# MIT-SPARK/BUFFER-X

Hardware: NVIDIA H100
Metric: registration pairs/sec (20k-pt clouds, 1500 kpts, 50k RANSAC) (higher is better)
Workload: dtype f32

## Files before the change

### buffer-x_b200/csrc/bx_conv_sd.cu

```cuda
#include <cuda_fp16.h>

#include "bx_common.cuh"
#include "bx_wgmma.cuh"

namespace {

constexpr int SD_BM = 128;
constexpr int SD_AROWS = 176;
constexpr int SD_SROWS = 176;
constexpr int SD_KBYTES = SD_AROWS * 16;
constexpr int SD_CHUNK = 4 * SD_KBYTES;
constexpr int SD_NL = 3;
constexpr int SD_NC = 8;
constexpr int SD_WGT_WARP = SD_NC + 3;
constexpr int SD_MAXNA = 12, SD_MAXNBS = 24;
constexpr int SD_TRING = 32;
constexpr int SD_SMEM = 227 * 1024 - 2048;

struct ConvSdParams {
    const float *in;
    const __half *w;
    const float *bias;
    float *out;
    int *flag;
    int n, Cout, nchunks, is3d, S_in, G_in, relu, n_tiles, NA;
    const int *d_n;
    const float *fa, *fb;
    int cyl, rs, W, OD, OW, S_out, rs_out;
    const __half *in_sd;
    __half *out_sd;
    long long rows_in, rows_out;
    int nbs;
    int resident;
    int *tile_ctr;
};

template <int NT, int IN_SD> struct SdCfg {
    static constexpr int NB = (NT == 128 && !IN_SD) ? 64 : NT;
    static constexpr int NH = NT / NB;
    static constexpr int SB = NT < 64 ? NT : 64;
    static constexpr int THREADS = (SD_NC + 4) * 32;
    static constexpr int PROD_REGS = IN_SD ? 56 : 136, MMA_REGS = IN_SD ? 224 : 184;
    static constexpr int B_STAGE = 3 * 64 * NT;
    static constexpr int STAGE_BYTES = SD_BM * SB * 4;
};
static_assert(128 * SdCfg<64, 1>::PROD_REGS + 256 * SdCfg<64, 1>::MMA_REGS == 384 * 168, "register split of the presplit kernels");
static_assert(128 * SdCfg<64, 0>::PROD_REGS + 256 * SdCfg<64, 0>::MMA_REGS == 384 * 168, "register split of the fp32-input kernels");

template <int R> __device__ __forceinline__ void setmaxnreg_inc() { asm volatile("setmaxnreg.inc.sync.aligned.u32 %0;" ::"n"(R)); }
template <int R> __device__ __forceinline__ void setmaxnreg_dec() { asm volatile("setmaxnreg.dec.sync.aligned.u32 %0;" ::"n"(R)); }

template <int CW, int OUT_SD, class Get8>
__device__ __forceinline__ void sd_store_rows(const ConvSdParams &p, int t, int row, int co0, int n_samples, Get8 get8) {
    const uint32_t R = (uint32_t)t * SD_BM + (uint32_t)row;
    const uint32_t s = R / (uint32_t)p.rs, q = R - s * (uint32_t)p.rs;
    const uint32_t y = q / (uint32_t)p.W, x = q - y * (uint32_t)p.W;
    const bool live = (int)s < n_samples;
    const bool valid = live && (int)y < p.OD && (int)x < p.OW;
    if constexpr (!OUT_SD) {
        if (!valid) return;
        const int S_out = p.S_out;
        float4 *eo = reinterpret_cast<float4 *>(p.out) + ((size_t)s * (p.Cout >> 2) + (co0 >> 2)) * S_out + (y * p.OW + x);
#pragma unroll
        for (int c = 0; c < CW; c += 8) {
            float r[8];
            get8(c, r);
#pragma unroll
            for (int e = 0; e < 8; ++e) r[e] = p.relu ? fmaxf(r[e], 0.0f) : r[e];
            if (co0 + c < p.Cout) eo[(size_t)(c >> 2) * S_out] = make_float4(r[0], r[1], r[2], r[3]);
            if (co0 + c + 4 < p.Cout) eo[(size_t)((c >> 2) + 1) * S_out] = make_float4(r[4], r[5], r[6], r[7]);
        }
    } else {
        const bool wz = p.cyl && live && ((y == 7 && x <= 20) || (y == 6 && x == 21));
        const bool z0 = p.cyl && R < 22;
        if (!valid && !wz && !z0) return;
        const size_t rows = (size_t)p.rows_out;
        const size_t pmain = p.cyl ? (size_t)R + 23 : (size_t)s * p.rs_out + y * p.OW + x;
        const long long pdup = !p.cyl ? -1 : (x == 19 ? (long long)R + 3 : (x == 0 ? (long long)R + 43 : -1));
        uint4 *img = reinterpret_cast<uint4 *>(p.out_sd) + (size_t)((co0 >> 4) * 4 + ((co0 >> 3) & 1)) * rows;
        const uint4 z = make_uint4(0u, 0u, 0u, 0u);
        float omax = 0.0f;
#pragma unroll
        for (int c = 0; c < CW; c += 8) {
            if (co0 + c < p.Cout) {
                if (valid) {
                    float r[8];
                    get8(c, r);
                    uint32_t hi[4], lo[4];
#pragma unroll
                    for (int e = 0; e < 4; ++e) {
                        float a = r[2 * e], b = r[2 * e + 1];
                        if (p.relu) { a = fmaxf(a, 0.0f); b = fmaxf(b, 0.0f); }
                        const __half2 hh = __floats2half2_rn(a, b);
                        const float2 hf = __half22float2(hh);
                        const __half2 ll = __floats2half2_rn((a - hf.x) * 2048.0f, (b - hf.y) * 2048.0f);
                        hi[e] = *reinterpret_cast<const uint32_t *>(&hh);
                        lo[e] = *reinterpret_cast<const uint32_t *>(&ll);
                        omax = fmaxf(omax, fmaxf(fabsf(a), fabsf(b)));
                    }
                    const uint4 vh = make_uint4(hi[0], hi[1], hi[2], hi[3]), vl = make_uint4(lo[0], lo[1], lo[2], lo[3]);
                    img[pmain] = vh; img[2 * rows + pmain] = vl;
                    if (pdup >= 0) { img[pdup] = vh; img[2 * rows + pdup] = vl; }
                } else if (wz) { img[pmain] = z; img[2 * rows + pmain] = z; }
                if (z0) { img[R] = z; img[2 * rows + R] = z; }
            }
            img += (((co0 + c) >> 3) & 1) ? 3 * rows : rows;
        }
        if (!(omax < 65000.0f) && p.flag) atomicOr(p.flag, 1);
    }
}

template <int NT, int IN_SD, int OUT_SD>
__global__ void __launch_bounds__(SdCfg<NT, IN_SD>::THREADS, 1) conv_sd_kernel(const ConvSdParams p) {
    using C = SdCfg<NT, IN_SD>;
    constexpr int NB = C::NB, NH = C::NH, SB = C::SB, WGT_WARP = SD_WGT_WARP;
    constexpr int BAR_AFULL = 0, BAR_AEMPTY = SD_MAXNA, BAR_BFULL = 2 * SD_MAXNA, BAR_BEMPTY = BAR_BFULL + SD_MAXNBS;
    constexpr int BAR_TILE = BAR_BEMPTY + SD_MAXNBS, NBARS = BAR_TILE + SD_TRING;
    extern __shared__ __align__(128) unsigned char smem[];
    __shared__ __align__(8) unsigned long long bars[NBARS];
    __shared__ int tile_ring[SD_TRING];
    __shared__ __align__(16) float bias_s[128];

    const int tid = threadIdx.x, lane = tid & 31;
    const int warp = __shfl_sync(0xffffffffu, tid >> 5, 0);
    const int NA = p.NA, NBS = p.nbs, nchunks = p.nchunks;
    const bool resident = p.resident != 0;
    const int n_samples = p.d_n ? min(*p.d_n, p.n) : p.n;
    const int n_tiles = (int)(((long long)n_samples * p.rs + SD_BM - 1) / SD_BM);
    float *const stage = reinterpret_cast<float *>(smem + (size_t)NA * SD_CHUNK + (size_t)NBS * C::B_STAGE);

    if (tid == 0) {
        for (int s = 0; s < SD_MAXNA; ++s) {
            mbar_init(smem_u32(&bars[BAR_AFULL + s]), IN_SD ? 1 : SD_NL);
            mbar_init(smem_u32(&bars[BAR_AEMPTY + s]), SD_NC);
        }
        for (int s = 0; s < SD_MAXNBS; ++s) {
            mbar_init(smem_u32(&bars[BAR_BFULL + s]), 1);
            mbar_init(smem_u32(&bars[BAR_BEMPTY + s]), SD_NC);
        }
        for (int s = 0; s < SD_TRING; ++s) mbar_init(smem_u32(&bars[BAR_TILE + s]), 1);
        asm volatile("fence.mbarrier_init.release.cluster;" ::: "memory");
    }
    if (threadIdx.x < 128) bias_s[threadIdx.x] = (int)threadIdx.x < p.Cout ? __ldg(p.bias + threadIdx.x) : 0.0f;
    __syncthreads();
    uint32_t a_base = smem_u32(smem);
    uint32_t b_base = a_base + (uint32_t)NA * SD_CHUNK;
    uint32_t bar_base = smem_u32(&bars[0]);
    asm volatile("" : "+r"(a_base), "+r"(b_base), "+r"(bar_base));

    const bool dyn = IN_SD && p.tile_ctr != nullptr;
    auto tile_of = [&](uint32_t k) -> int {
        if (!dyn) { const long long t = (long long)blockIdx.x + (long long)k * gridDim.x; return t < n_tiles ? (int)t : -1; }
        mbar_wait(bar_base + 8u * (BAR_TILE + (k & (SD_TRING - 1))), (k / SD_TRING) & 1u);
        return tile_ring[k & (SD_TRING - 1)];
    };

    if (warp < SD_NC) {
        setmaxnreg_inc<C::MMA_REGS>();
        const int wg = warp >> 2, tl = tid & 127;
        const int r0 = wg * 64 + (warp & 3) * 16 + (lane >> 2);
        const int cq = 2 * (lane & 3);
        constexpr uint32_t DESC_HI = 128u >> 4;
        constexpr uint32_t A_LBO = ((uint32_t)SD_KBYTES >> 4) << 16;
        constexpr uint32_t B_LBO = ((uint32_t)(2 * NT * 16) >> 4) << 16;
        constexpr uint32_t A_SPLIT = (2u * SD_KBYTES) >> 4, B_TAP16 = (64u * NT) >> 4, B_LO16 = (uint32_t)(NT * 16) >> 4;
        const uint32_t a0 = ((a_base + (uint32_t)wg * 64u * 16u) >> 4) | A_LBO;
        const uint32_t b0 = (b_base >> 4) | B_LBO;
        const uint32_t Wrow = (uint32_t)p.W;
        float run[NT / 2], acc[NB];
        uint32_t slot = 0, a_par = 0, q = 0, k = 0;
        for (int t = tile_of(0); t >= 0; t = tile_of(++k)) {
#pragma unroll
            for (int i = 0; i < NT / 2; ++i) run[i] = bias_s[(i / (NB / 2)) * NB + 8 * ((i % (NB / 2)) >> 2) + cq + (i & 1)];
            for (int c = 0; c < nchunks; ++c) {
                mbar_wait(bar_base + 8u * (BAR_AFULL + slot), a_par);
                const uint32_t ac = a0 + slot * ((uint32_t)SD_CHUNK >> 4);
                const uint32_t q0 = resident ? (uint32_t)c * 3u : q;
#pragma unroll
                for (int h = 0; h < NH; ++h) {
                    wgmma_fence();
#pragma unroll
                    for (int g = 0; g < 3; ++g) {
                        const uint32_t sq = q0 + (uint32_t)g, sb = sq % (uint32_t)NBS;
                        if (h == 0) mbar_wait(bar_base + 8u * (BAR_BFULL + sb), resident ? 0u : (sq / (uint32_t)NBS) & 1u);
                        const uint32_t bg = b0 + sb * ((uint32_t)C::B_STAGE >> 4);
#pragma unroll
                        for (int tt = 0; tt < 3; ++tt) {
                            const uint32_t ah = ac + (uint32_t)g * Wrow + (uint32_t)tt, al = ah + A_SPLIT;
                            const uint32_t bh = bg + (uint32_t)tt * B_TAP16 + (uint32_t)(h * NB), bl = bh + B_LO16;
                            const uint32_t acc_on = (g == 0 && tt == 0) ? 0u : 1u;
                            wgmma_f16<NB>(acc, gmma_desc(ah, DESC_HI), gmma_desc(bh, DESC_HI), acc_on);
                            if constexpr (NT < 128) {
                                wgmma_f16<NB>(acc + NB / 2, gmma_desc(ah, DESC_HI), gmma_desc(bl, DESC_HI), acc_on);
                                wgmma_f16<NB>(acc + NB / 2, gmma_desc(al, DESC_HI), gmma_desc(bh, DESC_HI), 1u);
                            } else {
                                wgmma_f16<NB>(acc + NB / 2, gmma_desc(al, DESC_HI), gmma_desc(bh, DESC_HI), acc_on);
                                wgmma_f16<NB>(acc + NB / 2, gmma_desc(ah, DESC_HI), gmma_desc(bl, DESC_HI), 1u);
                            }
                        }
                    }
                    wgmma_commit();
                    wgmma_wait<0>();
                    wgmma_fence_regs<NB>(acc);
#pragma unroll
                    for (int i = 0; i < NB / 2; ++i) run[h * (NB / 2) + i] += fmaf(acc[NB / 2 + i], 0.00048828125f, acc[i]);
                }
                __syncwarp();
                if (lane == 0) {
                    mbar_arrive(bar_base + 8u * (BAR_AEMPTY + slot));
                    if (!resident)
                        for (int g = 0; g < 3; ++g) mbar_arrive(bar_base + 8u * (BAR_BEMPTY + (q0 + (uint32_t)g) % (uint32_t)NBS));
                }
                if (++slot == (uint32_t)NA) { slot = 0; a_par ^= 1u; }
                if (!resident) q += 3;
            }
#pragma unroll
            for (int h = 0; h < NT / SB; ++h) {
                asm volatile("bar.sync %0, 128;" ::"r"(1 + wg) : "memory");
#pragma unroll
                for (int i = 0; i < SB / 2; i += 2) {
                    const int col = 8 * (i >> 2) + cq, row = r0 + ((i & 2) ? 8 : 0);
                    *reinterpret_cast<float2 *>(stage + ((size_t)(col >> 2) * SD_BM + row) * 4 + (col & 3)) =
                        make_float2(run[h * (SB / 2) + i], run[h * (SB / 2) + i + 1]);
                }
                asm volatile("bar.sync %0, 128;" ::"r"(1 + wg) : "memory");
                const int row = wg * 64 + (tl & 63), cs = (tl >> 6) * (SB / 2);
                const float4 *st4 = reinterpret_cast<const float4 *>(stage);
                sd_store_rows<SB / 2, OUT_SD>(p, t, row, h * SB + cs, n_samples, [&](int cc, float (&r)[8]) {
                    const float4 u0 = st4[((cs + cc) >> 2) * SD_BM + row], u1 = st4[(((cs + cc) >> 2) + 1) * SD_BM + row];
                    r[0] = u0.x; r[1] = u0.y; r[2] = u0.z; r[3] = u0.w; r[4] = u1.x; r[5] = u1.y; r[6] = u1.z; r[7] = u1.w;
                });
            }
        }
    } else {
        setmaxnreg_dec<C::PROD_REGS>();
        if (warp < WGT_WARP) {
            if (IN_SD) {
                if (warp == SD_NC && lane == 0) {
                    uint32_t slot = 0, par = 0, round = 0;
                    for (uint32_t k = 0;; ++k) {
                        int t;
                        if (dyn) {
                            t = atomicAdd(p.tile_ctr, 1);
                            if (t >= n_tiles) t = -1;
                            tile_ring[k & (SD_TRING - 1)] = t;
                            mbar_arrive(bar_base + 8u * (BAR_TILE + (k & (SD_TRING - 1))));
                        } else {
                            t = tile_of(k);
                        }
                        if (t < 0) break;
                        for (int c = 0; c < nchunks; ++c) {
                            if (round) mbar_wait(bar_base + 8u * (BAR_AEMPTY + slot), par ^ 1u);
                            mbar_arrive_expect_tx(bar_base + 8u * (BAR_AFULL + slot), 4u * (uint32_t)SD_KBYTES);
                            const unsigned char *src = reinterpret_cast<const unsigned char *>(p.in_sd) + ((size_t)(c * 4) * p.rows_in + (size_t)t * SD_BM) * 16;
#pragma unroll
                            for (int im = 0; im < 4; ++im)
                                bulk_g2s(a_base + slot * (uint32_t)SD_CHUNK + (uint32_t)im * SD_KBYTES, src + (size_t)im * p.rows_in * 16, (uint32_t)SD_KBYTES,
                                         bar_base + 8u * (BAR_AFULL + slot));
                            if (++slot == (uint32_t)NA) { slot = 0; par ^= 1u; round = 1; }
                        }
                    }
                }
                __syncwarp();
            } else {
                constexpr int ITEMS = (2 * SD_AROWS + SD_NL * 32 - 1) / (SD_NL * 32);
                const int ltid = tid - SD_NC * 32;
                const float4 *in4 = reinterpret_cast<const float4 *>(p.in);
                float amax = 0.0f;
                float4 cur[ITEMS][2], nxt[ITEMS][2];
                auto issue = [&](int t, int c, float4 (&v)[ITEMS][2]) {
                    const long long p0 = (long long)t * SD_BM;
#pragma unroll
                    for (int m = 0; m < ITEMS; ++m) {
                        const int idx = ltid + m * SD_NL * 32;
                        v[m][0] = make_float4(0.f, 0.f, 0.f, 0.f);
                        v[m][1] = v[m][0];
                        if (idx < 2 * SD_AROWS) {
                            const int h = idx >= SD_AROWS ? 1 : 0, r = idx - h * SD_AROWS;
                            const long long pr = p0 + r;
                            const int s = (int)(pr / p.rs), q = (int)(pr - (long long)s * p.rs);
                            const int yp = q / 22, xp = q - yp * 22;
                            if (s < n_samples && (yp != 0 || !p.cyl) && !p.fa) {
                                const int xx = xp == 0 ? 19 : (xp == 21 ? 0 : xp - 1);
                                int pos = p.cyl ? (yp - 1) * 20 + xx : q, g0;
                                if (p.is3d) { pos += c * 140; g0 = h * 2; } else { g0 = c * 4 + h * 2; }
                                const float4 *src = in4 + ((size_t)s * p.G_in + g0) * p.S_in + pos;
                                v[m][0] = __ldg(src);
                                v[m][1] = __ldg(src + p.S_in);
                            }
                        }
                    }
                };
                int j = 0;
                int t = blockIdx.x, c = 0;
                if (t < n_tiles) issue(t, 0, cur);
                while (t < n_tiles) {
                    int tn = t, cn = c + 1;
                    if (cn == nchunks) { cn = 0; tn = t + gridDim.x; }
                    if (tn < n_tiles) issue(tn, cn, nxt);
                    const int slot = j % NA;
                    if (j >= NA) mbar_wait(bar_base + 8u * (BAR_AEMPTY + slot), (uint32_t)(((j / NA) - 1) & 1));
                    unsigned char *dst = smem + (size_t)slot * SD_CHUNK;
                    if (p.fa) {
                        const long long p0 = (long long)t * SD_BM;
                        const int kk = c >> 1, cb = (c & 1) * 4;
                        float4 va[ITEMS][2], vb[ITEMS][2];
#pragma unroll
                        for (int m = 0; m < ITEMS; ++m) {
                            const int idx = ltid + m * SD_NL * 32;
                            va[m][0] = va[m][1] = vb[m][0] = vb[m][1] = make_float4(0.f, 0.f, 0.f, 0.f);
                            if (idx < 2 * SD_AROWS) {
                                const int h = idx >= SD_AROWS ? 1 : 0, r = idx - h * SD_AROWS;
                                const long long pr = p0 + r;
                                const int s = (int)(pr / 324), q = (int)(pr - (long long)s * 324);
                                const int nn = q / 18, ll = q - nn * 18;
                                if (s < n_samples) {
                                    int sh = ll - nn;
                                    sh = sh < 0 ? sh + 20 : sh;
                                    const float4 *sa = reinterpret_cast<const float4 *>(p.fa) + ((size_t)s * 8 + cb + h * 2) * 60 + kk * 20 + sh;
                                    const float4 *sb = reinterpret_cast<const float4 *>(p.fb) + ((size_t)s * 8 + cb + h * 2) * 54 + kk * 18 + ll;
                                    va[m][0] = __ldg(sa); va[m][1] = __ldg(sa + 60);
                                    vb[m][0] = __ldg(sb); vb[m][1] = __ldg(sb + 54);
                                }
                            }
                        }
#pragma unroll
                        for (int m = 0; m < ITEMS; ++m) {
                            cur[m][0] = make_float4(fmaxf(va[m][0].x - vb[m][0].x, 0.f), fmaxf(va[m][0].y - vb[m][0].y, 0.f), fmaxf(va[m][0].z - vb[m][0].z, 0.f),
                                                    fmaxf(va[m][0].w - vb[m][0].w, 0.f));
                            cur[m][1] = make_float4(fmaxf(va[m][1].x - vb[m][1].x, 0.f), fmaxf(va[m][1].y - vb[m][1].y, 0.f), fmaxf(va[m][1].z - vb[m][1].z, 0.f),
                                                    fmaxf(va[m][1].w - vb[m][1].w, 0.f));
                        }
                    }
#pragma unroll
                    for (int m = 0; m < ITEMS; ++m) {
                        const int idx = ltid + m * SD_NL * 32;
                        if (idx < 2 * SD_AROWS) {
                            const int h = idx >= SD_AROWS ? 1 : 0, r = idx - h * SD_AROWS;
                            const float xs[8] = {cur[m][0].x, cur[m][0].y, cur[m][0].z, cur[m][0].w, cur[m][1].x, cur[m][1].y, cur[m][1].z, cur[m][1].w};
                            uint32_t hi[4], lo[4];
#pragma unroll
                            for (int e = 0; e < 4; ++e) {
                                const __half2 hh = __floats2half2_rn(xs[2 * e], xs[2 * e + 1]);
                                const float2 hf = __half22float2(hh);
                                const __half2 ll = __floats2half2_rn((xs[2 * e] - hf.x) * 2048.0f, (xs[2 * e + 1] - hf.y) * 2048.0f);
                                hi[e] = *reinterpret_cast<const uint32_t *>(&hh);
                                lo[e] = *reinterpret_cast<const uint32_t *>(&ll);
                                amax = fmaxf(amax, fmaxf(fabsf(xs[2 * e]), fabsf(xs[2 * e + 1])));
                            }
                            *reinterpret_cast<uint4 *>(dst + (size_t)h * SD_KBYTES + (size_t)r * 16) = make_uint4(hi[0], hi[1], hi[2], hi[3]);
                            *reinterpret_cast<uint4 *>(dst + (size_t)(2 + h) * SD_KBYTES + (size_t)r * 16) = make_uint4(lo[0], lo[1], lo[2], lo[3]);
                        }
                    }
                    asm volatile("fence.proxy.async.shared::cta;" ::: "memory");
                    __syncwarp();
                    if (lane == 0) mbar_arrive(bar_base + 8u * (BAR_AFULL + slot));
#pragma unroll
                    for (int m = 0; m < ITEMS; ++m) { cur[m][0] = nxt[m][0]; cur[m][1] = nxt[m][1]; }
                    t = tn; c = cn; ++j;
                }
                if (!(amax < 65000.0f) && p.flag) atomicOr(p.flag, 1);
            }
        } else {
            if (lane == 0) {
                const int n_st = nchunks * 3;
                uint32_t q = 0;
                for (uint32_t k = 0; tile_of(k) >= 0; ++k) {
                    if (resident && k >= 1) break;
                    for (int s = 0; s < n_st; ++s, ++q) {
                        const uint32_t sb = q % (uint32_t)NBS, use = q / (uint32_t)NBS;
                        if (use > 0) mbar_wait(bar_base + 8u * (BAR_BEMPTY + sb), (use - 1) & 1u);
                        mbar_arrive_expect_tx(bar_base + 8u * (BAR_BFULL + sb), (uint32_t)C::B_STAGE);
                        bulk_g2s(b_base + sb * (uint32_t)C::B_STAGE, reinterpret_cast<const unsigned char *>(p.w) + (size_t)s * C::B_STAGE,
                                 (uint32_t)C::B_STAGE, bar_base + 8u * (BAR_BFULL + sb));
                    }
                }
            }
            __syncwarp();
        }
    }
    __syncthreads();
    if (dyn && tid == 0) {
        __threadfence();
        if (atomicAdd(p.tile_ctr + 1, 1) == (int)gridDim.x - 1) { p.tile_ctr[0] = 0; p.tile_ctr[1] = 0; __threadfence(); }
    }
}

template <int NT, int IN_SD, int OUT_SD>
int launch_sd(ConvSdParams p, cudaStream_t st) {
    using C = SdCfg<NT, IN_SD>;
    const int budget = SD_SMEM - C::STAGE_BYTES, n_st = p.nchunks * 3;
    p.resident = n_st <= SD_MAXNBS && budget - n_st * C::B_STAGE >= 3 * SD_CHUNK;
    p.nbs = p.resident ? n_st : 6;
    while (!p.resident && p.nbs > 3 && budget - p.nbs * C::B_STAGE < 4 * SD_CHUNK) --p.nbs;
    int na = (budget - p.nbs * C::B_STAGE) / SD_CHUNK;
    if (na > 2 * p.nchunks) na = 2 * p.nchunks;
    if (na > SD_MAXNA) na = SD_MAXNA;
    BX_REQUIRE(na >= 2, "bx_conv_layer_sd: no room for the activation ring");
    p.NA = na;
    const int smem = na * SD_CHUNK + p.nbs * C::B_STAGE + C::STAGE_BYTES;
    static BxPerDevice attr = {};
    if (bx_needs_attr(attr, (size_t)smem))
        BX_CUDA(cudaFuncSetAttribute(conv_sd_kernel<NT, IN_SD, OUT_SD>, cudaFuncAttributeMaxDynamicSharedMemorySize, smem));
    int sms = bx_device_sm_count();
    if (sms <= 0) sms = 132;
    const int grid = p.n_tiles < sms ? p.n_tiles : sms;
    conv_sd_kernel<NT, IN_SD, OUT_SD><<<grid, C::THREADS, smem, st>>>(p);
    BX_LAUNCH_CHECK();
    return BX_OK;
}

template <int NT>
int dispatch_sd(const ConvSdParams &p, int in_sd, int out_sd, cudaStream_t st) {
    if (in_sd) return out_sd ? launch_sd<NT, 1, 1>(p, st) : launch_sd<NT, 1, 0>(p, st);
    return out_sd ? launch_sd<NT, 0, 1>(p, st) : launch_sd<NT, 0, 0>(p, st);
}

}

BX_API long long bx_conv_sd_rows(int n, int rows_per_sample) {
    const long long rows = (long long)n * rows_per_sample;
    return (rows + SD_BM - 1) / SD_BM * SD_BM + (SD_AROWS - SD_BM);
}

BX_API int bx_conv_layer_sd(int geom, const void *in, int in_presplit, const void *w_sd, const float *bias, void *out, int out_presplit,
                            int n, const int32_t *d_n, int Cin, int Cout, int D, int W, int relu, int32_t *d_flag, int32_t *d_tile_ctr, void *stream) {
    BX_REQUIRE(in && w_sd && bias && out, "bx_conv_layer_sd: null pointer");
    BX_REQUIRE(geom == BX_GEOM_CYL3D || geom == BX_GEOM_CYL2D || geom == BX_GEOM_VALID3D, "bx_conv_layer_sd: geometry must be CYL3D, CYL2D or VALID3D (k = 3x1x3)");
    BX_REQUIRE(n >= 0 && Cin >= 16 && Cin % 16 == 0 && Cout >= 4 && Cout % 4 == 0 && Cout <= 128, "bx_conv_layer_sd: bad channels Cin=%d Cout=%d", Cin, Cout);
    BX_REQUIRE(geom != BX_GEOM_CYL3D || Cin == 16, "bx_conv_layer_sd: CYL3D expects 16 input channels x 3 radial slices");
    BX_REQUIRE(geom != BX_GEOM_VALID3D || (D >= 3 && W >= 3 && 2 * W + 2 <= SD_AROWS - SD_BM), "bx_conv_layer_sd: VALID3D raster %d x %d out of range (W <= 23)", D, W);
    BX_REQUIRE(!out_presplit || Cout % 16 == 0, "bx_conv_layer_sd: presplit output needs Cout %% 16 == 0");
    BX_REQUIRE(((reinterpret_cast<uintptr_t>(in) | reinterpret_cast<uintptr_t>(out) | reinterpret_cast<uintptr_t>(bias) | reinterpret_cast<uintptr_t>(w_sd)) & 15) == 0,
               "bx_conv_layer_sd: activations, weights and bias must be 16-byte aligned");
    if (n == 0) return BX_OK;
    ConvSdParams p = {};
    p.w = reinterpret_cast<const __half *>(w_sd); p.bias = bias; p.flag = d_flag; p.d_n = d_n; p.tile_ctr = d_tile_ctr;
    p.in = in_presplit ? nullptr : reinterpret_cast<const float *>(in);
    p.in_sd = in_presplit ? reinterpret_cast<const __half *>(in) : nullptr;
    p.out = out_presplit ? nullptr : reinterpret_cast<float *>(out);
    p.out_sd = out_presplit ? reinterpret_cast<__half *>(out) : nullptr;
    p.n = n; p.Cout = Cout; p.relu = relu;
    p.is3d = geom == BX_GEOM_CYL3D;
    p.cyl = geom != BX_GEOM_VALID3D;
    p.nchunks = p.is3d ? 3 : Cin / 16;
    p.G_in = Cin / 4;
    if (p.cyl) {
        p.rs = SD_SROWS; p.W = 22; p.OD = 7; p.OW = 20; p.S_out = 140; p.rs_out = SD_SROWS;
        p.S_in = p.is3d ? 420 : 140;
    } else {
        p.rs = D * W; p.W = W; p.OD = D - 2; p.OW = W - 2; p.S_out = p.OD * p.OW; p.rs_out = p.S_out;
        p.S_in = D * W;
    }
    const long long rows = (long long)n * p.rs;
    BX_REQUIRE(rows + 4 * SD_BM < 0x7fffffffLL, "bx_conv_layer_sd: too many samples (raster rows must stay below 2^31)");
    p.n_tiles = (int)((rows + SD_BM - 1) / SD_BM);
    p.rows_in = bx_conv_sd_rows(n, p.rs);
    p.rows_out = bx_conv_sd_rows(n, p.rs_out);
    cudaStream_t st = bx_stream(stream);
    if (Cout > 64) return dispatch_sd<128>(p, in_presplit, out_presplit, st);
    if (Cout > 32) return dispatch_sd<64>(p, in_presplit, out_presplit, st);
    return dispatch_sd<32>(p, in_presplit, out_presplit, st);
}

BX_API int bx_conv_layer_sd_costab(const float *fa, const float *fb, const void *w_sd, const float *bias, void *out, int out_presplit, int n,
                                   const int32_t *d_n, int relu, int32_t *d_flag, void *stream) {
    BX_REQUIRE(fa && fb && w_sd && bias && out, "bx_conv_layer_sd_costab: null pointer");
    BX_REQUIRE(((reinterpret_cast<uintptr_t>(fa) | reinterpret_cast<uintptr_t>(fb) | reinterpret_cast<uintptr_t>(out) | reinterpret_cast<uintptr_t>(bias) |
                 reinterpret_cast<uintptr_t>(w_sd)) & 15) == 0, "bx_conv_layer_sd_costab: pointers must be 16-byte aligned");
    if (n <= 0) return BX_OK;
    ConvSdParams p = {};
    p.w = reinterpret_cast<const __half *>(w_sd); p.bias = bias; p.flag = d_flag; p.d_n = d_n;
    p.fa = fa; p.fb = fb;
    p.in = fa;
    p.out = out_presplit ? nullptr : reinterpret_cast<float *>(out);
    p.out_sd = out_presplit ? reinterpret_cast<__half *>(out) : nullptr;
    p.n = n; p.Cout = 64; p.relu = relu;
    p.is3d = 0; p.cyl = 0; p.nchunks = 6; p.G_in = 8;
    p.rs = 324; p.W = 18; p.OD = 16; p.OW = 16; p.S_out = 256; p.rs_out = 256; p.S_in = 324;
    p.n_tiles = (int)(((long long)n * p.rs + SD_BM - 1) / SD_BM);
    p.rows_in = bx_conv_sd_rows(n, p.rs);
    p.rows_out = bx_conv_sd_rows(n, p.rs_out);
    return dispatch_sd<64>(p, 0, out_presplit, bx_stream(stream));
}
```

### buffer-x_b200/ops.py

```python
from __future__ import annotations

import ctypes
import os
from ctypes import c_double, c_float, c_int, c_int64, c_uint64, c_void_p

import numpy as np
import torch

_PKG = os.path.dirname(os.path.abspath(__file__))
LIB_PATH = os.path.join(_PKG, "libbufferx_b200.so")

SYMBOLS = [
    "bx_last_error", "bx_version", "bx_device_sm_count", "bx_launch_count", "bx_fps", "bx_radius_estimate", "bx_permute_cloud",
    "bx_select_patches", "bx_ball_query", "bx_lrf", "bx_spt_pnt", "bx_conv_layer", "bx_conv_tc_ntile", "bx_conv_layer_tc",
    "bx_pool_desc", "bx_mutual_nn",
    "bx_hypotheses", "bx_consensus", "bx_ransac_workspace_bytes", "bx_ransac", "bx_refine", "bx_conv_tc_set_segment_stages",
    "bx_radius_neighbors", "bx_grid_subsample", "bx_costvol_ab", "bx_concat_matches",
    "bx_pca_analysis", "bx_project_range", "bx_voxel_down_sample", "bx_conv_layer_sd", "bx_conv_sd_rows", "bx_spt_pnt_sd", "bx_fps_set_sync_mode", "bx_select_patches_seg", "bx_select_patches_workspace_bytes", "bx_conv_layer_sd_costab", "bx_lrf_batched", "bx_select_patches_batched", "bx_fps_ex", "bx_select_patches_grid", "bx_select_patches_grid_workspace_bytes", "bx_select_patches_grid_batched",
    "bx_gt_matches", "bx_so2_augment", "bx_equi_match", "bx_so2_gt",
]

GEOM_CYL3D, GEOM_CYL2D, GEOM_VALID3D, GEOM_COSTVOL, GEOM_COSTAB = 0, 1, 2, 3, 4
SELECT_PATCHES_SCAN = os.environ.get("BX_PATCHES", "scan").lower() != "seg"
RADIUS_BINS = 8192
# ... 289 lines not shown
                                         _dp(w, F32), _dp(b, F32), _dp(feat), _dp(vidx), _dp(inv), _stream()), "bx_spt_pnt")
    return (feat, vidx, inv) if debug else feat


def conv_layer(geom, x, w, bias, out, n, Cin, Cout, D, H, W, kd, kh, kw, relu, d_n=None, equi_s=None, equi_t=None,
               s_mids=None, t_mids=None):
    ev = None
    if profiler is not None and d_n is None:
        OD, OH, OW = (1, 7, 20) if geom in (GEOM_CYL3D, GEOM_CYL2D) else (D - kd + 1, H - kh + 1, W - kw + 1)
        ev = profiler.span("conv_desc", 2.0 * n * OD * OH * OW * Cout * Cin * kd * kh * kw)
        ev[0].record()
    elif profiler is not None:
        ev = profiler.span("conv_cost", 0.0)
        ev[0].record()
    _check(load_library().bx_conv_layer(geom, _dp(x, F32, "x"), _dp(w, F32, "w"), _dp(bias, F32, "bias"), _dp(out, F32, "out"), int(n),
                                        _dp(d_n, I32, "d_n"), Cin, Cout, D, H, W, kd, kh, kw, int(bool(relu)), _dp(equi_s, F32), _dp(equi_t, F32),
                                        _dp(s_mids, I32), _dp(t_mids, I32), _stream()), "bx_conv_layer")
    if ev:
        ev[1].record()
    return out


def tf32_split(w: torch.Tensor):
    bits = w.contiguous().view(torch.int32).to(torch.int64) & 0xFFFFFFFF
    hi_bits = ((bits + 0x1000) & 0xFFFFE000) & 0xFFFFFFFF
    hi_bits = torch.where(hi_bits >= 0x80000000, hi_bits - 0x100000000, hi_bits).to(torch.int32)
    hi = hi_bits.view(torch.float32)
    return hi, w - hi


def conv_tc_weights(Wt: torch.Tensor) -> torch.Tensor:
    T, Cin, Cout = Wt.shape
    assert Cin % 16 == 0 and Cout <= 128
    NT = 128 if Cout > 64 else (64 if Cout > 32 else 32)
    W = torch.zeros((T, Cin, NT), dtype=torch.float32, device=Wt.device)
    W[:, :, :Cout] = Wt
    hi, lo = tf32_split(W)
    both = torch.stack([hi, lo], dim=0)
    both = both.view(2, T, Cin // 16, 2, 2, 4, NT)
    img = both.permute(2, 1, 3, 0, 4, 6, 5).contiguous()
    return img.view(-1)


def to_blocked(x: torch.Tensor) -> torch.Tensor:
    n, C = x.shape[0], x.shape[1]
    return x.reshape(n, C // 4, 4, -1).permute(0, 1, 3, 2).contiguous()


def from_blocked(x: torch.Tensor) -> torch.Tensor:
    n, G, S, _ = x.shape
    return x.permute(0, 1, 3, 2).reshape(n, G * 4, S).contiguous()


def conv_layer_tc(geom, x, w_tc, bias, out, n, Cin, Cout, D, H, W, kd, kh, kw, relu, d_n=None, equi_s=None, equi_t=None,
                  s_mids=None, t_mids=None):
    ev = None
    if profiler is not None and d_n is None:
        OD, OH, OW = (1, 7, 20) if geom in (GEOM_CYL3D, GEOM_CYL2D) else (D - kd + 1, H - kh + 1, W - kw + 1)
        ev = profiler.span("conv_desc", 2.0 * n * OD * OH * OW * Cout * Cin * kd * kh * kw)
        ev[0].record()
    elif profiler is not None:
        ev = profiler.span("conv_cost", 0.0)
        ev[0].record()
    _check(load_library().bx_conv_layer_tc(geom, _dp(x, F32, "x"), _dp(w_tc, F32, "w_tc"), _dp(bias, F32, "bias"), _dp(out, F32, "out"), int(n),
                                           _dp(d_n, I32, "d_n"), Cin, Cout, D, H, W, kd, kh, kw, int(bool(relu)), _dp(equi_s, F32), _dp(equi_t, F32),
                                           _dp(s_mids, I32), _dp(t_mids, I32), _stream()), "bx_conv_layer_tc")
    if ev:
        ev[1].record()
    return out


def conv_sd_weights(Wt: torch.Tensor) -> torch.Tensor:
    T, Cin, Cout = Wt.shape
    assert T in (9, 27) and Cin % 16 == 0 and Cout <= 128 and (T == 9 or Cin == 16)
    NT = 128 if Cout > 64 else (64 if Cout > 32 else 32)
    W = torch.zeros((T, Cin, NT), dtype=torch.float32, device=Wt.device)
    W[:, :, :Cout] = Wt
    if T == 27:
        W = W.view(3, 9, 16, NT)
    else:
        W = W.view(9, Cin // 16, 16, NT).permute(1, 0, 2, 3)
    hi = W.half()
    lo = ((W - hi.float()) * 2048.0).half()
    both = torch.stack([hi, lo], dim=2)
    nch = both.shape[0]
    both = both.reshape(nch, 9, 2, 2, 8, NT).permute(0, 1, 3, 2, 5, 4).contiguous()
    return both.view(-1)


def conv_sd_rows(n: int, rows_per_sample: int = 176) -> int:
    return int(load_library().bx_conv_sd_rows(int(n), int(rows_per_sample)))


def conv_sd_buffer(n: int, C: int, device, rows_per_sample: int = 176):
    return torch.empty((C // 16, 4, conv_sd_rows(n, rows_per_sample), 8), dtype=torch.float16, device=device)


def conv_layer_sd(geom, x, w_sd, bias, out, n, Cin, Cout, relu, flag=None, d_n=None, D=0, W=0, tile_ctr=None):
    ev = None
    if profiler is not None:
        if geom == GEOM_VALID3D:
            ev = profiler.span("conv_cost", 0.0)
        else:
            ev = profiler.span("conv_desc", 2.0 * n * 140 * Cout * Cin * (27 if geom == GEOM_CYL3D else 9))
        ev[0].record()
    in_sd, out_sd = x.dtype == torch.float16, out.dtype == torch.float16
    _check(load_library().bx_conv_layer_sd(geom, _dp(x, None, "x"), int(in_sd), _dp(w_sd, torch.float16, "w_sd"), _dp(bias, F32, "bias"),
                                           _dp(out, None, "out"), int(out_sd), int(n), _dp(d_n, I32, "d_n"), Cin, Cout, int(D), int(W), int(bool(relu)),
                                           _dp(flag, I32, "flag"), _dp(tile_ctr, I32, "tile_ctr"), _stream()), "bx_conv_layer_sd")
    if ev:
        ev[1].record()
    return out


def conv_sd_weights_costab(Wt: torch.Tensor) -> torch.Tensor:
    assert Wt.shape == (27, 32, 64)
    W = Wt.view(3, 3, 3, 32, 64).permute(1, 0, 2, 3, 4).reshape(3, 9, 32, 64)
    W = W.permute(1, 0, 2, 3).reshape(9, 96, 64).contiguous()
    return conv_sd_weights(W)


def conv_layer_sd_costab(fa, fb, w_sd, bias, out, n, relu, flag=None, d_n=None):
    ev = profiler.span("conv_cost", 0.0) if profiler is not None else None
    if ev:
        ev[0].record()
    _check(load_library().bx_conv_layer_sd_costab(_dp(fa, F32, "fa"), _dp(fb, F32, "fb"), _dp(w_sd, torch.float16, "w_sd"), _dp(bias, F32, "bias"),
                                                  _dp(out, None, "out"), int(out.dtype == torch.float16), int(n), _dp(d_n, I32, "d_n"), int(bool(relu)),
                                                  _dp(flag, I32, "flag"), _stream()), "bx_conv_layer_sd_costab")
    if ev:
        ev[1].record()
    return out


def sd_pack(x: torch.Tensor) -> torch.Tensor:
    n, C = x.shape[0], x.shape[1]
    rows = conv_sd_rows(n)
    xp = torch.zeros((n, C, 8, 22), dtype=torch.float32, device=x.device)
    xp[:, :, 1:, 1:21] = x
    xp[:, :, 1:, 0] = x[:, :, :, 19]
    xp[:, :, 1:, 21] = x[:, :, :, 0]
    flat = torch.zeros((rows, C), dtype=torch.float32, device=x.device)
    flat[: n * 176] = xp.permute(0, 2, 3, 1).reshape(n * 176, C)
    hi = flat.half()
    lo = ((flat - hi.float()) * 2048.0).half()
    img = torch.stack([hi, lo], dim=0).view(2, rows, C // 16, 2, 8).permute(2, 0, 3, 1, 4).contiguous()
    return img.view(C // 16, 4, rows, 8)


def sd_unpack(img: torch.Tensor, n: int) -> torch.Tensor:
    nch, _, rows, _ = img.shape
    v = img.view(nch, 2, 2, rows, 8).float()
    val = v[:, 0] + v[:, 1] / 2048.0
    flat = val.permute(2, 0, 1, 3).reshape(rows, nch * 16)
    xp = flat[: n * 176].view(n, 8, 22, nch * 16).permute(0, 3, 1, 2)
    return xp[:, :, 1:, 1:21].contiguous(), xp


def costvol_factor_weights(Wt: torch.Tensor):
    W = Wt.detach().double().cpu().view(3, 3, 3, Wt.shape[1], Wt.shape[2])
    wa = torch.zeros((Wt.shape[1], 3, 5, Wt.shape[2]), dtype=torch.float64)
    for dn in range(3):
        for dl in range(3):
            wa[:, :, dl - dn + 2, :] += W[dn, :, dl].permute(1, 0, 2)
    wb = W.sum(dim=0).permute(2, 0, 1, 3).contiguous()
    return wa.float().contiguous().to(Wt.device), wb.float().contiguous().to(Wt.device)


def costvol_ab(equi_s, equi_t, s_mids, t_mids, d_M, maxM, wa, wb, bias, A=None, B=None):
# ... 236 lines not shown
```

Before: 102.9.

## Swap wgmma operands for narrow presplit convs so weights fill the M dimension

For the presplit-input conv with Cout of 64 or less, the weights now act as the wgmma A operand (M=64 channels) and activations as B (N=128 rows). Each warpgroup handles its own 128-row tile, so a block processes two tiles per work unit, and the activation ring, barriers and grid are sized per unit. For Cout=32 the weights are repacked on the host into a hi/lo plus zero/hi block layout so that one N=128 instruction pair covers the split-precision product. This is meant to avoid narrow-N wgmma shapes that waste tensor-core throughput. The cost is more complex indexing, an extra staging layout, and a partially idle warpgroup on an odd tile count.

```diff
diff --git a/buffer-x_b200/csrc/bx_conv_sd.cu b/buffer-x_b200/csrc/bx_conv_sd.cu
--- a/buffer-x_b200/csrc/bx_conv_sd.cu
+++ b/buffer-x_b200/csrc/bx_conv_sd.cu
@@ -36,12 +36,15 @@
 };
 
 template <int NT, int IN_SD> struct SdCfg {
+    static constexpr bool CM = IN_SD && NT < 128;
+    static constexpr int TPU = CM ? 2 : 1;
     static constexpr int NB = (NT == 128 && !IN_SD) ? 64 : NT;
     static constexpr int NH = NT / NB;
     static constexpr int SB = NT < 64 ? NT : 64;
     static constexpr int THREADS = (SD_NC + 4) * 32;
     static constexpr int PROD_REGS = IN_SD ? 56 : 136, MMA_REGS = IN_SD ? 224 : 184;
-    static constexpr int B_STAGE = 3 * 64 * NT;
+    static constexpr int WR = NT < 64 ? 64 : NT;
+    static constexpr int B_STAGE = 3 * 64 * WR;
     static constexpr int STAGE_BYTES = SD_BM * SB * 4;
 };
 static_assert(128 * SdCfg<64, 1>::PROD_REGS + 256 * SdCfg<64, 1>::MMA_REGS == 384 * 168, "register split of the presplit kernels");
@@ -127,12 +130,13 @@
     const bool resident = p.resident != 0;
     const int n_samples = p.d_n ? min(*p.d_n, p.n) : p.n;
     const int n_tiles = (int)(((long long)n_samples * p.rs + SD_BM - 1) / SD_BM);
+    const int n_units = (n_tiles + C::TPU - 1) / C::TPU;
     float *const stage = reinterpret_cast<float *>(smem + (size_t)NA * SD_CHUNK + (size_t)NBS * C::B_STAGE);
 
     if (tid == 0) {
         for (int s = 0; s < SD_MAXNA; ++s) {
             mbar_init(smem_u32(&bars[BAR_AFULL + s]), IN_SD ? 1 : SD_NL);
-            mbar_init(smem_u32(&bars[BAR_AEMPTY + s]), SD_NC);
+            mbar_init(smem_u32(&bars[BAR_AEMPTY + s]), C::CM ? 4 : SD_NC);
         }
         for (int s = 0; s < SD_MAXNBS; ++s) {
             mbar_init(smem_u32(&bars[BAR_BFULL + s]), 1);
@@ -150,7 +154,7 @@
 
     const bool dyn = IN_SD && p.tile_ctr != nullptr;
     auto tile_of = [&](uint32_t k) -> int {
-        if (!dyn) { const long long t = (long long)blockIdx.x + (long long)k * gridDim.x; return t < n_tiles ? (int)t : -1; }
+        if (!dyn) { const long long t = (long long)blockIdx.x + (long long)k * gridDim.x; return t < n_units ? (int)t : -1; }
         mbar_wait(bar_base + 8u * (BAR_TILE + (k & (SD_TRING - 1))), (k / SD_TRING) & 1u);
         return tile_ring[k & (SD_TRING - 1)];
     };
@@ -158,106 +162,193 @@
     if (warp < SD_NC) {
         setmaxnreg_inc<C::MMA_REGS>();
         const int wg = warp >> 2, tl = tid & 127;
-        const int r0 = wg * 64 + (warp & 3) * 16 + (lane >> 2);
-        const int cq = 2 * (lane & 3);
         constexpr uint32_t DESC_HI = 128u >> 4;
         constexpr uint32_t A_LBO = ((uint32_t)SD_KBYTES >> 4) << 16;
-        constexpr uint32_t B_LBO = ((uint32_t)(2 * NT * 16) >> 4) << 16;
-        constexpr uint32_t A_SPLIT = (2u * SD_KBYTES) >> 4, B_TAP16 = (64u * NT) >> 4, B_LO16 = (uint32_t)(NT * 16) >> 4;
-        const uint32_t a0 = ((a_base + (uint32_t)wg * 64u * 16u) >> 4) | A_LBO;
-        const uint32_t b0 = (b_base >> 4) | B_LBO;
+        constexpr uint32_t A_SPLIT = (2u * SD_KBYTES) >> 4;
+        constexpr uint32_t B_LBO = ((uint32_t)(2 * C::WR * 16) >> 4) << 16, B_TAP16 = (64u * C::WR) >> 4;
         const uint32_t Wrow = (uint32_t)p.W;
-        float run[NT / 2], acc[NB];
         uint32_t slot = 0, a_par = 0, q = 0, k = 0;
-        for (int t = tile_of(0); t >= 0; t = tile_of(++k)) {
-#pragma unroll
-            for (int i = 0; i < NT / 2; ++i) run[i] = bias_s[(i / (NB / 2)) * NB + 8 * ((i % (NB / 2)) >> 2) + cq + (i & 1)];
-            for (int c = 0; c < nchunks; ++c) {
-                mbar_wait(bar_base + 8u * (BAR_AFULL + slot), a_par);
-                const uint32_t ac = a0 + slot * ((uint32_t)SD_CHUNK >> 4);
+        if constexpr (C::CM) {
+            constexpr int NACC = NT == 64 ? 128 : 64;
+            constexpr uint32_t W_LO16 = (64u * 16u) >> 4;
+            const int wq = warp & 3;
+            auto ch = [&](int i) { return NT == 64 ? 16 * wq + (lane >> 2) + 8 * ((i & 3) >> 1) : 8 * wq + (lane >> 2); };
+            auto col = [&](int i) { return (NT == 64 ? 8 * (i >> 2) : 8 * (i >> 1)) + 2 * (lane & 3) + (i & 1); };
+            auto mi = [](int i) { return NT == 64 ? i : 4 * (i >> 1) + (i & 1); };
+            auto xi = [](int i) { return NT == 64 ? 64 + i : 4 * (i >> 1) + 2 + (i & 1); };
+            const uint32_t x0 = ((a_base + (uint32_t)wg * SD_CHUNK) >> 4) | A_LBO;
+            const uint32_t w0 = (b_base >> 4) | B_LBO;
+            const uint32_t nslots = (uint32_t)NA / 2u;
+            float run[NT], acc[NACC];
+            auto chunk = [&](int c) {
+                const uint32_t cs = 2u * slot + (uint32_t)wg;
+                mbar_wait(bar_base + 8u * (BAR_AFULL + cs), a_par);
+                const uint32_t xc = x0 + slot * ((2u * SD_CHUNK) >> 4);
                 const uint32_t q0 = resident ? (uint32_t)c * 3u : q;
-#pragma unroll
-                for (int h = 0; h < NH; ++h) {
-                    wgmma_fence();
-#pragma unroll
-                    for (int g = 0; g < 3; ++g) {
-                        const uint32_t sq = q0 + (uint32_t)g, sb = sq % (uint32_t)NBS;
-                        if (h == 0) mbar_wait(bar_base + 8u * (BAR_BFULL + sb), resident ? 0u : (sq / (uint32_t)NBS) & 1u);
-                        const uint32_t bg = b0 + sb * ((uint32_t)C::B_STAGE >> 4);
-#pragma unroll
-                        for (int tt = 0; tt < 3; ++tt) {
-                            const uint32_t ah = ac + (uint32_t)g * Wrow + (uint32_t)tt, al = ah + A_SPLIT;
-                            const uint32_t bh = bg + (uint32_t)tt * B_TAP16 + (uint32_t)(h * NB), bl = bh + B_LO16;
-                            const uint32_t acc_on = (g == 0 && tt == 0) ? 0u : 1u;
-                            wgmma_f16<NB>(acc, gmma_desc(ah, DESC_HI), gmma_desc(bh, DESC_HI), acc_on);
-                            if constexpr (NT < 128) {
-                                wgmma_f16<NB>(acc + NB / 2, gmma_desc(ah, DESC_HI), gmma_desc(bl, DESC_HI), acc_on);
-                                wgmma_f16<NB>(acc + NB / 2, gmma_desc(al, DESC_HI), gmma_desc(bh, DESC_HI), 1u);
-                            } else {
-                                wgmma_f16<NB>(acc + NB / 2, gmma_desc(al, DESC_HI), gmma_desc(bh, DESC_HI), acc_on);
-                                wgmma_f16<NB>(acc + NB / 2, gmma_desc(ah, DESC_HI), gmma_desc(bl, DESC_HI), 1u);
-                            }
-                        }
-                    }
-                    wgmma_commit();
-                    wgmma_wait<0>();
-                    wgmma_fence_regs<NB>(acc);
-#pragma unroll
-                    for (int i = 0; i < NB / 2; ++i) run[h * (NB / 2) + i] += fmaf(acc[NB / 2 + i], 0.00048828125f, acc[i]);
-                }
+                wgmma_fence();
+#pragma unroll
+                for (int g = 0; g < 3; ++g) {
+                    const uint32_t sq = q0 + (uint32_t)g, sb = sq % (uint32_t)NBS;
+                    mbar_wait(bar_base + 8u * (BAR_BFULL + sb), resident ? 0u : (sq / (uint32_t)NBS) & 1u);
+                    const uint32_t wgt = w0 + sb * ((uint32_t)C::B_STAGE >> 4);
+#pragma unroll
+                    for (int tt = 0; tt < 3; ++tt) {
+                        const uint32_t xh = xc + (uint32_t)g * Wrow + (uint32_t)tt, xl = xh + A_SPLIT;
+                        const uint32_t wh = wgt + (uint32_t)tt * B_TAP16, wl = wh + W_LO16;
+                        const uint32_t acc_on = (g == 0 && tt == 0) ? 0u : 1u;
+                        if constexpr (NT == 64) {
+                            wgmma_f16<128>(acc, gmma_desc(wh, DESC_HI), gmma_desc(xh, DESC_HI), acc_on);
+                            wgmma_f16<128>(acc + 64, gmma_desc(wl, DESC_HI), gmma_desc(xh, DESC_HI), acc_on);
+                            wgmma_f16<128>(acc + 64, gmma_desc(wh, DESC_HI), gmma_desc(xl, DESC_HI), 1u);
+                        } else {
+                            wgmma_f16<128>(acc, gmma_desc(wh, DESC_HI), gmma_desc(xh, DESC_HI), acc_on);
+                            wgmma_f16<128>(acc, gmma_desc(wl, DESC_HI), gmma_desc(xl, DESC_HI), 1u);
+                        }
+                    }
+                }
+                wgmma_commit();
+                wgmma_wait<0>();
+                wgmma_fence_regs<NACC>(acc);
+#pragma unroll
+                for (int i = 0; i < NT; ++i) run[i] += fmaf(acc[xi(i)], 0.00048828125f, acc[mi(i)]);
                 __syncwarp();
                 if (lane == 0) {
-                    mbar_arrive(bar_base + 8u * (BAR_AEMPTY + slot));
+                    mbar_arrive(bar_base + 8u * (BAR_AEMPTY + cs));
                     if (!resident)
                         for (int g = 0; g < 3; ++g) mbar_arrive(bar_base + 8u * (BAR_BEMPTY + (q0 + (uint32_t)g) % (uint32_t)NBS));
                 }
-                if (++slot == (uint32_t)NA) { slot = 0; a_par ^= 1u; }
+                if (++slot == nslots) { slot = 0; a_par ^= 1u; }
                 if (!resident) q += 3;
+            };
+            float *const st = stage + (size_t)wg * 64 * NT;
+            const float4 *st4 = reinterpret_cast<const float4 *>(st);
+            for (int u = tile_of(0); u >= 0; u = tile_of(++k)) {
+#pragma unroll
+                for (int i = 0; i < NT; ++i) run[i] = bias_s[ch(i)];
+                for (int c = 0; c < nchunks; c += 2) {
+                    chunk(c);
+                    if (c + 1 < nchunks) chunk(c + 1);
+                }
+                const int t = 2 * u + wg;
+                if (t >= n_tiles) continue;
+#pragma unroll
+                for (int h = 0; h < 2; ++h) {
+                    asm volatile("bar.sync %0, 128;" ::"r"(1 + wg) : "memory");
+#pragma unroll
+                    for (int i = 0; i < NT; ++i)
+                        if ((col(i) >> 6) == h) st[((ch(i) >> 2) * 64 + (col(i) & 63)) * 4 + (ch(i) & 3)] = run[i];
+                    asm volatile("bar.sync %0, 128;" ::"r"(1 + wg) : "memory");
+                    const int row = tl & 63, cs = (tl >> 6) * (NT / 2);
+                    sd_store_rows<NT / 2, OUT_SD>(p, t, h * 64 + row, cs, n_samples, [&](int cc, float (&r)[8]) {
+                        const float4 u0 = st4[((cs + cc) >> 2) * 64 + row], u1 = st4[(((cs + cc) >> 2) + 1) * 64 + row];
+                        r[0] = u0.x; r[1] = u0.y; r[2] = u0.z; r[3] = u0.w; r[4] = u1.x; r[5] = u1.y; r[6] = u1.z; r[7] = u1.w;
+                    });
+                }
             }
-#pragma unroll
-            for (int h = 0; h < NT / SB; ++h) {
-                asm volatile("bar.sync %0, 128;" ::"r"(1 + wg) : "memory");
-#pragma unroll
-                for (int i = 0; i < SB / 2; i += 2) {
-                    const int col = 8 * (i >> 2) + cq, row = r0 + ((i & 2) ? 8 : 0);
-                    *reinterpret_cast<float2 *>(stage + ((size_t)(col >> 2) * SD_BM + row) * 4 + (col & 3)) =
-                        make_float2(run[h * (SB / 2) + i], run[h * (SB / 2) + i + 1]);
-                }
-                asm volatile("bar.sync %0, 128;" ::"r"(1 + wg) : "memory");
-                const int row = wg * 64 + (tl & 63), cs = (tl >> 6) * (SB / 2);
-                const float4 *st4 = reinterpret_cast<const float4 *>(stage);
-                sd_store_rows<SB / 2, OUT_SD>(p, t, row, h * SB + cs, n_samples, [&](int cc, float (&r)[8]) {
-                    const float4 u0 = st4[((cs + cc) >> 2) * SD_BM + row], u1 = st4[(((cs + cc) >> 2) + 1) * SD_BM + row];
-                    r[0] = u0.x; r[1] = u0.y; r[2] = u0.z; r[3] = u0.w; r[4] = u1.x; r[5] = u1.y; r[6] = u1.z; r[7] = u1.w;
-                });
-            }
+        } else {
+            const int r0 = wg * 64 + (warp & 3) * 16 + (lane >> 2);
+            const int cq = 2 * (lane & 3);
+            constexpr uint32_t B_DESC_HI = (NT < 64 ? 256u : 128u) >> 4, B_LO16 = (NT < 64 ? 128u : (uint32_t)NT * 16u) >> 4;
+            const uint32_t a0 = ((a_base + (uint32_t)wg * 64u * 16u) >> 4) | A_LBO;
+            const uint32_t b0 = (b_base >> 4) | B_LBO;
+            float run[NT / 2], acc[NB];
+            for (int t = tile_of(0); t >= 0; t = tile_of(++k)) {
+#pragma unroll
+                for (int i = 0; i < NT / 2; ++i) run[i] = bias_s[(i / (NB / 2)) * NB + 8 * ((i % (NB / 2)) >> 2) + cq + (i & 1)];
+                for (int c = 0; c < nchunks; ++c) {
+                    mbar_wait(bar_base + 8u * (BAR_AFULL + slot), a_par);
+                    const uint32_t ac = a0 + slot * ((uint32_t)SD_CHUNK >> 4);
+                    const uint32_t q0 = resident ? (uint32_t)c * 3u : q;
+#pragma unroll
+                    for (int h = 0; h < NH; ++h) {
+                        wgmma_fence();
+#pragma unroll
+                        for (int g = 0; g < 3; ++g) {
+                            const uint32_t sq = q0 + (uint32_t)g, sb = sq % (uint32_t)NBS;
+                            if (h == 0) mbar_wait(bar_base + 8u * (BAR_BFULL + sb), resident ? 0u : (sq / (uint32_t)NBS) & 1u);
+                            const uint32_t bg = b0 + sb * ((uint32_t)C::B_STAGE >> 4);
+#pragma unroll
+                            for (int tt = 0; tt < 3; ++tt) {
+                                const uint32_t ah = ac + (uint32_t)g * Wrow + (uint32_t)tt, al = ah + A_SPLIT;
+                                const uint32_t bh = bg + (uint32_t)tt * B_TAP16 + (uint32_t)(h * NB), bl = bh + B_LO16;
+                                const uint32_t acc_on = (g == 0 && tt == 0) ? 0u : 1u;
+                                wgmma_f16<NB>(acc, gmma_desc(ah, DESC_HI), gmma_desc(bh, B_DESC_HI), acc_on);
+                                if constexpr (NT < 128) {
+                                    wgmma_f16<NB>(acc + NB / 2, gmma_desc(ah, DESC_HI), gmma_desc(bl, B_DESC_HI), acc_on);
+                                    wgmma_f16<NB>(acc + NB / 2, gmma_desc(al, DESC_HI), gmma_desc(bh, B_DESC_HI), 1u);
+                                } else {
+                                    wgmma_f16<NB>(acc + NB / 2, gmma_desc(al, DESC_HI), gmma_desc(bh, B_DESC_HI), acc_on);
+                                    wgmma_f16<NB>(acc + NB / 2, gmma_desc(ah, DESC_HI), gmma_desc(bl, B_DESC_HI), 1u);
+                                }
+                            }
+                        }
+                        wgmma_commit();
+                        wgmma_wait<0>();
+                        wgmma_fence_regs<NB>(acc);
+#pragma unroll
+                        for (int i = 0; i < NB / 2; ++i) run[h * (NB / 2) + i] += fmaf(acc[NB / 2 + i], 0.00048828125f, acc[i]);
+                    }
+                    __syncwarp();
+                    if (lane == 0) {
+                        mbar_arrive(bar_base + 8u * (BAR_AEMPTY + slot));
+                        if (!resident)
+                            for (int g = 0; g < 3; ++g) mbar_arrive(bar_base + 8u * (BAR_BEMPTY + (q0 + (uint32_t)g) % (uint32_t)NBS));
+                    }
+                    if (++slot == (uint32_t)NA) { slot = 0; a_par ^= 1u; }
+                    if (!resident) q += 3;
+                }
+#pragma unroll
+                for (int h = 0; h < NT / SB; ++h) {
+                    asm volatile("bar.sync %0, 128;" ::"r"(1 + wg) : "memory");
+#pragma unroll
+                    for (int i = 0; i < SB / 2; i += 2) {
+                        const int col = 8 * (i >> 2) + cq, row = r0 + ((i & 2) ? 8 : 0);
+                        *reinterpret_cast<float2 *>(stage + ((size_t)(col >> 2) * SD_BM + row) * 4 + (col & 3)) =
+                            make_float2(run[h * (SB / 2) + i], run[h * (SB / 2) + i + 1]);
+                    }
+                    asm volatile("bar.sync %0, 128;" ::"r"(1 + wg) : "memory");
+                    const int row = wg * 64 + (tl & 63), cs = (tl >> 6) * (SB / 2);
+                    const float4 *st4 = reinterpret_cast<const float4 *>(stage);
+                    sd_store_rows<SB / 2, OUT_SD>(p, t, row, h * SB + cs, n_samples, [&](int cc, float (&r)[8]) {
+                        const float4 u0 = st4[((cs + cc) >> 2) * SD_BM + row], u1 = st4[(((cs + cc) >> 2) + 1) * SD_BM + row];
+                        r[0] = u0.x; r[1] = u0.y; r[2] = u0.z; r[3] = u0.w; r[4] = u1.x; r[5] = u1.y; r[6] = u1.z; r[7] = u1.w;
+                    });
+                }
+        }
         }
     } else {
         setmaxnreg_dec<C::PROD_REGS>();
         if (warp < WGT_WARP) {
             if (IN_SD) {
                 if (warp == SD_NC && lane == 0) {
+                    constexpr uint32_t TPU = C::TPU;
+                    const uint32_t nslots = (uint32_t)NA / TPU;
                     uint32_t slot = 0, par = 0, round = 0;
                     for (uint32_t k = 0;; ++k) {
-                        int t;
+                        int u;
                         if (dyn) {
-                            t = atomicAdd(p.tile_ctr, 1);
-                            if (t >= n_tiles) t = -1;
-                            tile_ring[k & (SD_TRING - 1)] = t;
+                            u = atomicAdd(p.tile_ctr, 1);
+                            if (u >= n_units) u = -1;
+                            tile_ring[k & (SD_TRING - 1)] = u;
                             mbar_arrive(bar_base + 8u * (BAR_TILE + (k & (SD_TRING - 1))));
                         } else {
-                            t = tile_of(k);
-                        }
-                        if (t < 0) break;
+                            u = tile_of(k);
+                        }
+                        if (u < 0) break;
                         for (int c = 0; c < nchunks; ++c) {
-                            if (round) mbar_wait(bar_base + 8u * (BAR_AEMPTY + slot), par ^ 1u);
-                            mbar_arrive_expect_tx(bar_base + 8u * (BAR_AFULL + slot), 4u * (uint32_t)SD_KBYTES);
-                            const unsigned char *src = reinterpret_cast<const unsigned char *>(p.in_sd) + ((size_t)(c * 4) * p.rows_in + (size_t)t * SD_BM) * 16;
-#pragma unroll
-                            for (int im = 0; im < 4; ++im)
-                                bulk_g2s(a_base + slot * (uint32_t)SD_CHUNK + (uint32_t)im * SD_KBYTES, src + (size_t)im * p.rows_in * 16, (uint32_t)SD_KBYTES,
-                                         bar_base + 8u * (BAR_AFULL + slot));
-                            if (++slot == (uint32_t)NA) { slot = 0; par ^= 1u; round = 1; }
+#pragma unroll
+                            for (uint32_t g = 0; g < TPU; ++g) {
+                                const uint32_t cs = slot * TPU + g;
+                                const int t = (int)(TPU * (uint32_t)u + g) < n_tiles ? (int)(TPU * (uint32_t)u + g) : (int)(TPU * (uint32_t)u);
+                                if (round) mbar_wait(bar_base + 8u * (BAR_AEMPTY + cs), par ^ 1u);
+                                mbar_arrive_expect_tx(bar_base + 8u * (BAR_AFULL + cs), 4u * (uint32_t)SD_KBYTES);
+                                const unsigned char *src = reinterpret_cast<const unsigned char *>(p.in_sd) + ((size_t)(c * 4) * p.rows_in + (size_t)t * SD_BM) * 16;
+#pragma unroll
+                                for (int im = 0; im < 4; ++im)
+                                    bulk_g2s(a_base + cs * (uint32_t)SD_CHUNK + (uint32_t)im * SD_KBYTES, src + (size_t)im * p.rows_in * 16, (uint32_t)SD_KBYTES,
+                                             bar_base + 8u * (BAR_AFULL + cs));
+                            }
+                            if (++slot == nslots) { slot = 0; par ^= 1u; round = 1; }
                         }
                     }
                 }
@@ -390,13 +481,14 @@
 int launch_sd(ConvSdParams p, cudaStream_t st) {
     using C = SdCfg<NT, IN_SD>;
     const int budget = SD_SMEM - C::STAGE_BYTES, n_st = p.nchunks * 3;
-    p.resident = n_st <= SD_MAXNBS && budget - n_st * C::B_STAGE >= 3 * SD_CHUNK;
+    p.resident = n_st <= SD_MAXNBS && budget - n_st * C::B_STAGE >= (C::CM ? 4 : 3) * SD_CHUNK;
     p.nbs = p.resident ? n_st : 6;
     while (!p.resident && p.nbs > 3 && budget - p.nbs * C::B_STAGE < 4 * SD_CHUNK) --p.nbs;
     int na = (budget - p.nbs * C::B_STAGE) / SD_CHUNK;
-    if (na > 2 * p.nchunks) na = 2 * p.nchunks;
+    if (na > 2 * C::TPU * p.nchunks) na = 2 * C::TPU * p.nchunks;
     if (na > SD_MAXNA) na = SD_MAXNA;
-    BX_REQUIRE(na >= 2, "bx_conv_layer_sd: no room for the activation ring");
+    na -= na % C::TPU;
+    BX_REQUIRE(na >= 2 * C::TPU, "bx_conv_layer_sd: no room for the activation ring");
     p.NA = na;
     const int smem = na * SD_CHUNK + p.nbs * C::B_STAGE + C::STAGE_BYTES;
     static BxPerDevice attr = {};
@@ -404,7 +496,8 @@
         BX_CUDA(cudaFuncSetAttribute(conv_sd_kernel<NT, IN_SD, OUT_SD>, cudaFuncAttributeMaxDynamicSharedMemorySize, smem));
     int sms = bx_device_sm_count();
     if (sms <= 0) sms = 132;
-    const int grid = p.n_tiles < sms ? p.n_tiles : sms;
+    const int units = (p.n_tiles + C::TPU - 1) / C::TPU;
+    const int grid = units < sms ? units : sms;
     conv_sd_kernel<NT, IN_SD, OUT_SD><<<grid, C::THREADS, smem, st>>>(p);
     BX_LAUNCH_CHECK();
     return BX_OK;
diff --git a/buffer-x_b200/ops.py b/buffer-x_b200/ops.py
--- a/buffer-x_b200/ops.py
+++ b/buffer-x_b200/ops.py
@@ -395,8 +395,14 @@
         W = W.view(9, Cin // 16, 16, NT).permute(1, 0, 2, 3)
     hi = W.half()
     lo = ((W - hi.float()) * 2048.0).half()
+    nch = W.shape[0]
+    if NT == 32:
+        grp = lambda x: x.reshape(nch, 9, 2, 8, 4, 8).permute(0, 1, 2, 4, 5, 3)
+        h, l = grp(hi), grp(lo)
+        P = torch.stack([h, l], dim=4)
+        Q = torch.stack([torch.zeros_like(h), h], dim=4)
+        return torch.stack([P, Q], dim=3).contiguous().view(-1)
     both = torch.stack([hi, lo], dim=2)
-    nch = both.shape[0]
     both = both.reshape(nch, 9, 2, 2, 8, NT).permute(0, 1, 3, 2, 5, 4).contiguous()
     return both.view(-1)
 
```

New measurement: 108.8 (median of 6 runs). 5.8% higher.
